# GIJaws/gym-simpletetris

Measured on AMD Instinct MI355X. Metric: env-steps/sec at 65 536 parallel 10×20 boards; 1→8 GPU scaling, higher is better.
Workload: dtype u32

## Files before the change

gym-simpletetris_amd/csrc/st_kernels.hip:

```cpp
#include "st_internal.h"


namespace st {
namespace {

constexpr int kShapes[7][4][2] = {
    {{0, 0}, {-1, 0}, {1, 0}, {0, -1}},   {{0, 0}, {-1, 0}, {0, -1}, {0, -2}},
    {{0, 0}, {1, 0}, {0, -1}, {0, -2}},   {{0, 0}, {-1, 0}, {0, -1}, {1, -1}},
    {{0, 0}, {-1, -1}, {0, -1}, {1, 0}},  {{0, 0}, {0, -1}, {0, -2}, {0, -3}},
    {{0, 0}, {0, -1}, {-1, 0}, {-1, -1}},
};

struct PieceTab {
    uint32_t m[28], g[28];
    bool ok;
};

constexpr PieceTab make_piece_tab() {
    PieceTab t{};
    t.ok = true;
    for (int p = 0; p < 7; ++p) {
        int cx[4] = {}, cy[4] = {};
        for (int c = 0; c < 4; ++c) {
            cx[c] = kShapes[p][c][0];
// ... 30 lines not shown
                const int i = cx[c], j = cy[c];
                cx[c] = j;
                cy[c] = -i;
            }
        }
    }
    return t;
}
constexpr PieceTab kTab = make_piece_tab();
static_assert(kTab.ok, "every tetromino column must be a contiguous run within [-3, 3]");
#define ST_TAB28(a) {a[0], a[1], a[2], a[3], a[4], a[5], a[6], a[7], a[8], a[9], a[10], a[11], \
                     a[12], a[13], a[14], a[15], a[16], a[17], a[18], a[19], a[20], a[21], a[22], \
                     a[23], a[24], a[25], a[26], a[27]}
__constant__ uint32_t c_tab_m[28] = ST_TAB28(kTab.m);
__constant__ uint32_t c_tab_g[28] = ST_TAB28(kTab.g);

constexpr PieceTab make_box_tab() {
    PieceTab t{};
    t.ok = true;
    for (int p = 0; p < 7; ++p) {
        int cx[4] = {}, cy[4] = {};
        for (int c = 0; c < 4; ++c) {
            cx[c] = kShapes[p][c][0];
            cy[c] = kShapes[p][c][1];
        }
        for (int r = 0; r < 4; ++r) {
            int dx0 = 99, dx1 = -99;
            for (int c = 0; c < 4; ++c) {
                dx0 = cx[c] < dx0 ? cx[c] : dx0;
                dx1 = cx[c] > dx1 ? cx[c] : dx1;
            }
            if (dx0 < -3 || dx0 > 0 || dx1 - dx0 > 3) t.ok = false;
            uint32_t m = 0, g = (uint32_t)(dx0 + 3);
            for (int k = 0; k < 4; ++k) g |= 64u << (3 + 7 * k);
            for (int k = 0; k < 4; ++k) {
                int ymin = 99, ymax = -99, cnt = 0;
                uint32_t bits = 0;
                for (int c = 0; c < 4; ++c)
                    if (cx[c] == dx0 + k) {
                        ++cnt;
                        ymin = cy[c] < ymin ? cy[c] : ymin;
                        ymax = cy[c] > ymax ? cy[c] : ymax;
                        bits |= 1u << (cy[c] + 3);
                    }
                if (!cnt) continue;
                if (cnt != ymax - ymin + 1 || ymin < -3 || ymax > 3) t.ok = false;
                m |= bits << (8 * k);
                g = (g & ~(127u << (3 + 7 * k))) | ((uint32_t)(ymax + 1) & 127u) << (3 + 7 * k);
            }
            t.m[p * 4 + r] = m;
            t.g[p * 4 + r] = g;
            for (int c = 0; c < 4; ++c) {
                const int i = cx[c], j = cy[c];
                cx[c] = j;
                cy[c] = -i;
            }
        }
    }
    return t;
}
constexpr PieceTab kBox = make_box_tab();
static_assert(kBox.ok, "every rotation must span at most four columns from dx0 in [-3, 0]");

__device__ __forceinline__ int pc_dx(uint32_t g, int j) { return (int)((g >> (6 * j)) & 7u) - 3; }
__device__ __forceinline__ int pc_bot(uint32_t g, int j) { return (int)((g >> (6 * j + 3)) & 7u) - 3; }
template <bool S32 = false>
__device__ __forceinline__ uint32_t pc_bits(uint32_t m, int j, int y) {
    if constexpr (S32) return (((m >> (8 * j)) & 0xFFu) << y) >> 3;
    return (uint32_t)((uint64_t)((m >> (8 * j)) & 0xFFu) << y >> 3);
}

typedef int i32x4 __attribute__((ext_vector_type(4)));
constexpr uint32_t kOff = 0xFFFFFFF0u;
__device__ __forceinline__ __amdgpu_buffer_rsrc_t buf_rsrc(const void *base, uint32_t bytes) {
    return __builtin_amdgcn_make_buffer_rsrc(const_cast<void *>(base), 0, base ? (int)bytes : 0,
                                             0x00020000);
}
constexpr int kNT = 2;
constexpr int kST = kNT;
constexpr int kRD = kNT;
constexpr int kDrawPrio = 2;
constexpr int kLogicPrio = 1;
template <int AUX = 0>
__device__ __forceinline__ void buf_store16(__amdgpu_buffer_rsrc_t r, uint32_t off, uint4 v) {
    const i32x4 d = {(int)v.x, (int)v.y, (int)v.z, (int)v.w};
    __builtin_amdgcn_raw_buffer_store_b128(d, r, off, 0, AUX);
}

__device__ __forceinline__ uint32_t &lcol(uint32_t *L, int x, int lane) {
    return L[(x + kPad) * kWave + lane];
}

__device__ __forceinline__ void read_cols(const uint32_t *L, int lane, uint32_t g, int x,
                                          uint32_t (&v)[4]) {
#pragma unroll
    for (int j = 0; j < 4; ++j) v[j] = L[(x + pc_dx(g, j) + kPad) * kWave + lane];
}
template <bool S32 = false>
__device__ __forceinline__ bool collides_v(uint32_t m, int y, const uint32_t (&v)[4]) {
    uint32_t hit = 0;
#pragma unroll
    for (int j = 0; j < 4; ++j) hit |= pc_bits<S32>(m, j, y) & v[j];
    return hit != 0;
}
__device__ __forceinline__ int drop_v(uint32_t g, int y, const uint32_t (&v)[4]) {
    int dist = 1 << 20;
#pragma unroll
    for (int j = 0; j < 4; ++j) {
        const int yb = y + pc_bot(g, j);
        const int s = yb + 1 > 0 ? yb + 1 : 0;
        const int k = __builtin_ctz(v[j] & (~0u << s)) - yb - 1;
        dist = k < dist ? k : dist;
    }
    return dist;
}

template <bool S32 = false>
__device__ __forceinline__ void paint(uint32_t *L, int lane, uint32_t m, uint32_t g, int x, int y,
                                      uint32_t hmask) {
#pragma unroll
    for (int j = 0; j < 4; ++j)
        atomicOr(&L[(x + pc_dx(g, j) + kPad) * kWave + lane], pc_bits<S32>(m, j, y) & hmask);
}

template <bool S32 = false>
__device__ __forceinline__ void erase(uint32_t *L, int lane, uint32_t m, uint32_t g, int x, int y,
                                      uint32_t hmask) {
#pragma unroll
    for (int j = 0; j < 4; ++j)
        atomicAnd(&L[(x + pc_dx(g, j) + kPad) * kWave + lane], ~(pc_bits<S32>(m, j, y) & hmask));
}

__device__ __forceinline__ int box_x0(uint32_t g, int x) { return x + (int)(g & 7u) - 3; }
__device__ __forceinline__ void read_box(const uint32_t *L, int lane, uint32_t g, int x, uint32_t (&v)[4]) {
    const uint32_t *c0 = &L[(box_x0(g, x) + kPad) * kWave + lane];
#pragma unroll
    for (int j = 0; j < 4; ++j) v[j] = c0[j * kWave];
}
__device__ __forceinline__ int drop_box(uint32_t g, int y, const uint32_t (&v)[4]) {
    int dist = 0;
#pragma unroll
    for (int j = 0; j < 4; ++j) {
        const int q = y + ((int32_t)(g << (32 - 10 - 7 * j)) >> 25);
        const int s = q > 0 ? q : 0;
        const int k = __builtin_ctz(v[j] & (~0u << s)) - q;
        dist = j == 0 || k < dist ? k : dist;
    }
    return dist;
}
template <bool S32 = false>
__device__ __forceinline__ void paint_box(uint32_t *L, int lane, uint32_t m, uint32_t g, int x, int y,
                                          uint32_t hmask) {
    uint32_t *c0 = &L[(box_x0(g, x) + kPad) * kWave + lane];
#pragma unroll
    for (int j = 0; j < 4; ++j) atomicOr(&c0[j * kWave], pc_bits<S32>(m, j, y) & hmask);
}
template <bool S32 = false>
__device__ __forceinline__ void erase_box(uint32_t *L, int lane, uint32_t m, uint32_t g, int x, int y,
                                          uint32_t hmask) {
    uint32_t *c0 = &L[(box_x0(g, x) + kPad) * kWave + lane];
#pragma unroll
    for (int j = 0; j < 4; ++j) atomicAnd(&c0[j * kWave], ~(pc_bits<S32>(m, j, y) & hmask));
}

__device__ __forceinline__ uint32_t compact(uint32_t v, uint32_t full) {
    while (full) {
        const int r = __builtin_ctz(full);
        full &= full - 1u;
        const uint32_t above = (1u << r) - 1u;
        v = (v & ~(above | (1u << r))) | ((v & above) << 1);
    }
    return v;
}

__device__ __forceinline__ void wave_sync() {
    __builtin_amdgcn_fence(__ATOMIC_RELEASE, "wavefront");
    __builtin_amdgcn_wave_barrier();
    __builtin_amdgcn_fence(__ATOMIC_ACQUIRE, "wavefront");
}

__device__ __forceinline__ uint32_t mt_temper(uint32_t y) {
    y ^= (y >> 11);
    y = __builtin_amdgcn_bitop3_b32(y, y << 7, 0x9d2c5680u, 0x78);
    y = __builtin_amdgcn_bitop3_b32(y, y << 15, 0xefc60000u, 0x78);
    y ^= (y >> 18);
    return y;
}
__device__ __forceinline__ uint32_t mt_temper_hi18(uint32_t y) {
    y ^= (y >> 11);
    y = __builtin_amdgcn_bitop3_b32(y, y << 7, 0x9d2c5680u, 0x78);
    return __builtin_amdgcn_bitop3_b32(y, y << 15, 0xefc60000u, 0x78);
}
__device__ __forceinline__ uint32_t mt_mix(uint32_t a, uint32_t b) {
    const uint32_t y = (a & 0x80000000u) | (b & 0x7fffffffu);
    return (y >> 1) ^ ((y & 1u) ? 0x9908b0dfu : 0u);
}

constexpr uint32_t kMtB = kMtN;
constexpr uint32_t kMtPad = 2 * kMtN;
constexpr int kMtWin = 16;
__device__ __forceinline__ void mt_unpack(uint32_t r, int &idx, int &pg, int &cur) {
    idx = (int)(r & 0x3FFu);
    pg = (int)((r >> 10) & 0x3FFu);
    cur = (int)((r >> 20) & 1u);
}
__device__ __forceinline__ uint32_t mt_pack(int idx, int pg, int cur) {
    return (uint32_t)idx | ((uint32_t)pg << 10) | ((uint32_t)cur << 20);
}
constexpr uint32_t kMtLow = (1u << 21) - 1u;
constexpr uint32_t kPvOk = 1u << 24;
constexpr uint32_t kPvCMax = 63u;
__device__ __forceinline__ uint32_t mt_keep(uint32_t hi, uint32_t low) { return (hi & ~kMtLow) | low; }
__device__ __forceinline__ int pv_id(uint32_t r) { return (int)((r >> 21) & 7u); }
// ... 445 lines not shown
    [[maybe_unused]] uint64_t draw_kind = 0;
    constexpr bool S32 = HT != 0 && HT <= 25;
    const uint32_t kFlags = SC0 ? (p.flags & (ST_REWARD_STEP | ST_STEP_RESET)) : p.flags;

#if defined(ST_ABLATION) && ST_ABLATION
    const uint32_t kAblate = p.ablate;
#else
    constexpr uint32_t kAblate = 0u;
#endif
    [[maybe_unused]] uint64_t rt0 = 0;
    if constexpr (STAMP) {
        rt0 = __builtin_amdgcn_s_memrealtime();
        tlast = __builtin_amdgcn_s_memtime();
    }
    ST_STAMP(0);
    if constexpr (ROLE == kRoleL && KSTEPS == 1) __builtin_amdgcn_s_setprio(kLogicPrio);
    uint32_t *const L = sm.L;
    uint32_t *const SS = sm.SS;
    const int W = WT ? WT : p.W;
    const int H = HT ? HT : p.H;
    const int lane = threadIdx.x & (kWave - 1);
    const int64_t e0 = (int64_t)blockIdx.x * kWave;
    const int64_t e = e0 + lane;
    const int64_t sd = p.stride;
    const bool real = e < p.n;
    const uint32_t hmask = (1u << H) - 1u;
    const uint32_t floorb = ~hmask;

    const uint32_t loff = (uint32_t)(lane >> 4) * (uint32_t)sd + 4u * (uint32_t)(lane & 15);
    constexpr int NBQ = ((WT ? WT : kMaxW) + 3) / 4;
    const uint32_t *bsrc = p.board + e0;
    const uint32_t *ssrc = reinterpret_cast<const uint32_t *>(p.stats) + ((kAblate & 1024u) ? 0 : e0);
    constexpr bool OVP = KSTEPS == 1;
    constexpr bool LCL = KSTEPS == 1 && !VEC;
    static_assert(ST_STAT_MT_INDEX == ST_STAT_COUNT0 + 7, "counts and MT word: 8 consecutive rows");
    auto mine_q = [&](int q) {
        if constexpr (LCL) return ROLE == kRoleD && (q == 1 || q == 2);
        return (ROLE == kRoleL) == (q < 2);
    };
    auto qbase = [&](int q) -> int {
        if constexpr (LCL) return ST_STAT_COUNT0 + 4 * (q - 1);
        return 4 * q;
    };
    auto clamp_off = [&](int q, int nrows) -> uint32_t {
        const int r = 4 * q + (lane >> 4) < nrows ? (lane >> 4) : nrows - 1 - 4 * q;
        return (uint32_t)r * (uint32_t)sd + 4u * (uint32_t)(lane & 15);
    };
    uint4 bv[NBQ];
    if constexpr (DO_L) {
#pragma unroll
        for (int q = 0; q < NBQ; ++q)
            if (WT || 4 * q < W)
                bv[q] = *reinterpret_cast<const uint4 *>(bsrc + (size_t)(4 * q) * sd +
                                                         (4 * q + 4 <= W ? loff : clamp_off(q, W)));
    }
    static_assert(kHotQ == 4, "four staged counter groups");
    uint4 sv0 = make_uint4(0u, 0u, 0u, 0u), sv1 = sv0, sv2 = sv0, sv3 = sv0;
    auto ldq = [&](int q) -> uint4 {
        return *reinterpret_cast<const uint4 *>(ssrc + (size_t)qbase(q) * sd +
                                                (qbase(q) + 4 <= kHotRows ? loff : clamp_off(q, kHotRows)));
    };
    if (mine_q(0)) sv0 = ldq(0);
    if (mine_q(1) && !(LCL && (kAblate & 262144u))) sv1 = ldq(1);
    if (mine_q(2)) sv2 = ldq(2);
    if (mine_q(3)) sv3 = ldq(3);
    const int K = KSTEPS ? KSTEPS : p.k;
    constexpr bool STEP2 = KSTEPS == 1;
    constexpr bool ACT = DO_L;
    uint32_t act_next = 0;
    if constexpr (ACT) act_next = p.actions[real ? e : p.n - 1];
    [[maybe_unused]] uint32_t gate_v = 0;
    if constexpr (VEC) gate_v = __builtin_amdgcn_raw_buffer_load_b32(buf_rsrc(p.gate, 4u), 0u, 0, 0);
    constexpr bool DL = KSTEPS == 1 && ROLE == kRoleL;
    [[maybe_unused]] uint32_t pw_d = 0, tm_d = 0;
    if constexpr (DL) {
        pw_d = p.piece[e];
        tm_d = reinterpret_cast<const uint32_t *>(p.stats)[(int64_t)ST_STAT_TIME * sd + e];
    }
    constexpr bool BUILD = DO_D;
    uint32_t tab_m = 0, tab_g = 0;
    if constexpr (BUILD) {
#pragma unroll
        for (int i = 0; i < 28; ++i) {
            asm("v_writelane_b32 %0, %1, %2" : "+v"(tab_m) : "s"(kTab.m[i]), "i"(i));
            asm("v_writelane_b32 %0, %1, %2" : "+v"(tab_g) : "s"(kTab.g[i]), "i"(i));
        }
    }
    const int lrow = lane >> 4, lcc = 4 * (lane & 15);
    if constexpr (DO_L) {
#pragma unroll
        for (int q = 0; q < NBQ; ++q) {
            if (WT || 4 * q < W) {
                uint4 v = bv[q];
                v.x |= floorb;
                v.y |= floorb;
                v.z |= floorb;
                v.w |= floorb;
                uint32_t *dst = &L[(4 * q + lrow + kPad) * kWave + lcc];
                if constexpr (ROLE == kRoleL) dst = 4 * q + lrow < W ? dst : &sm.dump[lcc];
                *reinterpret_cast<uint4 *>(dst) = v;
            }
        }
    }
    if constexpr (BUILD) {
#pragma unroll
        for (int x = 0; x < kPad; ++x) {
            L[x * kWave + lane] = ~0u;
            L[(W + kPad + x) * kWave + lane] = ~0u;
        }
        if (lane < 28) {
            sm.T2[2 * lane] = tab_m;
            sm.T2[2 * lane + 1] = tab_g;
        }
        if constexpr (F32) {
            if (lane < 16) {
                sm.F4[4 * lane] = (float)(lane & 1);
                sm.F4[4 * lane + 1] = (float)((lane >> 1) & 1);
                sm.F4[4 * lane + 2] = (float)((lane >> 2) & 1);
                sm.F4[4 * lane + 3] = (float)((lane >> 3) & 1);
            }
        }
    }
    auto stq = [&](int q, const uint4 &v) { *reinterpret_cast<uint4 *>(&SS[(qbase(q) + lrow) * kWave + lcc]) = v; };
    if (mine_q(0)) stq(0, sv0);
    if (mine_q(1)) stq(1, sv1);
    if (mine_q(2)) stq(2, sv2);
    if (mine_q(3)) stq(3, sv3);
    if constexpr (OVP && DO_L) {
#pragma unroll
        for (int q = 0; q < NBQ; ++q)
            if ((WT || 4 * q < W) && 4 * q + lrow < W)
                *reinterpret_cast<uint4 *>(&sm.OV[(4 * q + lrow + kPad) * kWave + lcc]) = make_uint4(0u, 0u, 0u, 0u);
    }
    if (ROLE == kRoleL && lane == 0) sm.f1 = 0u;
    if (ROLE == kRoleD && lane == 0) sm.f2 = 0u;
    wg_barrier();
    if constexpr (VEC) {
        if (p.gate && __builtin_amdgcn_readfirstlane(gate_v) == p.gate_epoch) return;
    }
    auto ss = [&](int r) -> uint32_t & { return SS[r * kWave + lane]; };
    auto tab = [&](int i) -> uint2 { return *reinterpret_cast<const uint2 *>(&sm.T2[2 * i]); };
    [[maybe_unused]] bool bad_act = false;
    for (int t = 0; t < K; ++t) {
    uint32_t act = 6u;
    if constexpr (ACT) {
        act = real ? act_next : 6u;
        bad_act |= act > 6u;
        if (KSTEPS != 1 && t + 1 < K) act_next = p.actions[(int64_t)(t + 1) * p.n + (real ? e : p.n - 1)];
    }
    uint32_t *const obs_t = p.obs ? p.obs + (int64_t)t * W * p.n : nullptr;
    const uint32_t pw = DL ? pw_d : ss(kPieceRow);
    int32_t time = (int32_t)(DL ? tm_d : ss(ST_STAT_TIME));
    const int id = (int)(pw & 7u);
    int rot = (int)((pw >> 3) & 3u);
    int ax = (int)((pw >> 5) & 63u);
    int ay = (int)((pw >> 11) & 63u);
    int lock = (int)(pw >> 17);
    uint32_t mt0 = ss(ST_STAT_MT_INDEX);
    if constexpr (STAMP && KSTEPS == 1) asm volatile("s_waitcnt vmcnt(0) lgkmcnt(0)" ::: "memory");
    ST_STAMP(1);

    uint2 desc = make_uint2(0u, 0u);
    bool locknow = false;
    int32_t rew = 0;
    [[maybe_unused]] uint2 pd_pv = make_uint2(0u, 0u);
    if constexpr (ACT) {
        const bool tries = act == 0u || act == 1u || act == 4u || act == 5u;
        const int cx = ax + (act == 0u ? -1 : (act == 1u ? 1 : 0));
        const int cr = (rot + (act == 4u ? 1 : 0) + (act == 5u ? 3 : 0)) & 3;
        desc = tab(id * 4 + rot);
        const uint2 cdesc = tab(id * 4 + cr);
        if constexpr (OVP && DO_L) pd_pv = tab(pv_id(mt0) * 4);
        uint32_t cur[4], cand[4];
        read_cols(L, lane, desc.y, ax, cur);
        read_cols(L, lane, cdesc.y, cx, cand);
        const bool ok = tries && !collides_v<S32>(cdesc.x, ay, cand);
        ax = ok ? cx : ax;
        rot = ok ? cr : rot;
        desc.x = ok ? cdesc.x : desc.x;
        desc.y = ok ? cdesc.y : desc.y;
#pragma unroll
        for (int j = 0; j < 4; ++j) cur[j] = ok ? cand[j] : cur[j];
        int d = drop_v(desc.y, ay, cur);
        if (act == 2u) {
            ay += d;
            d = 0;
        } else if (act == 3u && d > 0) {
            ay += 1;
            d -= 1;
        }
        if (d > 0) {
            ay += 1;
            d -= 1;
            if (kFlags & ST_STEP_RESET) lock = 0;
        }
        time += 1;
        rew = (kFlags & ST_REWARD_STEP) ? 1 : 0;
        if (d == 0) {
            const int l1 = lock + 1;
            lock = lock_next(l1, p.lock_mod);
            locknow = lock == 0 && !(kAblate & 1u);
        }
    }
    ST_STAMP(2);
    [[maybe_unused]] uint32_t lcv[5] = {};
    if constexpr (LCL && DO_L) {
        const auto rs = buf_rsrc(p.stats, (uint32_t)kHotRows * (uint32_t)sd * 4u);
        const uint32_t eo = (kAblate & 8192u) ? (uint32_t)lane * 4u : (uint32_t)e * 4u;
#pragma unroll
        for (int j = 0; j < 5; ++j)
            lcv[j] = __builtin_amdgcn_raw_buffer_load_b32(
                rs, locknow && !(kAblate & 2097152u) ? eo + (uint32_t)(ST_STAT_SCORE + j) * (uint32_t)sd * 4u : kOff,
                0, 0);
    }
    [[maybe_unused]] MtChunk chunk;
    [[maybe_unused]] MtRes mrs;
    [[maybe_unused]] int32_t cnt[7];
    [[maybe_unused]] DrawPar dpar;
    [[maybe_unused]] int32_t csid = 0;
    if constexpr (DO_D) {
        mrs = mt_res(p.mt + e0 * kMtPitch, lane);
        mt_chunk_issue(mrs, mt0, real && !(kAblate & (2u | 1048576u)), lane, chunk);
        const int s0 = pv_id(mt0);
#pragma unroll
        for (int i = 0; i < 7; ++i) cnt[i] = (int32_t)ss(ST_STAT_COUNT0 + i) + (i == s0);
        csid = cnt[0];
#pragma unroll
        for (int i = 1; i < 7; ++i) csid = s0 == i ? cnt[i] : csid;
        dpar = draw_par(cnt);
    }
    if constexpr (DO_L) {
        const uint64_t m = __ballot(locknow);
        if (lane == 0) {
            sm.lockm[t & 1][0] = (uint32_t)m;
            sm.lockm[t & 1][1] = (uint32_t)(m >> 32);
        }
    }
    wg_barrier();
    if constexpr (DO_D || KSTEPS != 1) ST_STAMP(10);
    if constexpr (DO_D) __builtin_amdgcn_s_setprio(kDrawPrio);
    if constexpr (DO_D) {
        const uint32_t w = lane < 32 ? sm.lockm[t & 1][0] : sm.lockm[t & 1][1];
        locknow = (w >> (lane & 31)) & 1u;
    }
    if constexpr (DO_L && KSTEPS != 1) {
        if (t > 0) mt0 = sm.mtw[(t - 1) & 1][lane];
    }

    uint32_t mtst = mt0;
    const bool want_pre = locknow && !(kAblate & 2u);
    constexpr int kWin = STEP2 ? 8 : 16;
    MtPre pre;
    if constexpr (DO_D) mt_pre_load<kWin>(mrs, mtst, want_pre && !(kAblate & 524288u), pre);

    [[maybe_unused]] const bool wide_obs1 = OVP && (p.n & 3) == 0 && e0 + kWave <= p.n &&
                                            (reinterpret_cast<uintptr_t>(p.obs) & 15u) == 0 &&
                                            (!VEC || (reinterpret_cast<uintptr_t>(p.final_obs) & 15u) == 0);

    bool died = false, spawn = false;
    int32_t score = 0, lines = 0, holes = 0, height = 0, deaths = 0;
    int32_t o_score = 0, o_lines = 0, o_holes = 0, o_height = 0, o_deaths = 0;
    [[maybe_unused]] bool hset = false;
    uint32_t bdirty = 0;
    if (DO_L && locknow) {
        if constexpr (!LCL) {
            score = o_score = (int32_t)ss(ST_STAT_SCORE);
            lines = o_lines = (int32_t)ss(ST_STAT_LINES);
            holes = o_holes = (int32_t)ss(ST_STAT_HOLES);
            height = o_height = (int32_t)ss(ST_STAT_PIECE_HEIGHT);
            deaths = o_deaths = (int32_t)ss(ST_STAT_DEATHS);
        }
        paint<S32>(L, lane, desc.x, desc.y, ax, ay, hmask);
        uint32_t andv = ~0u, orv = 0, sctz = 0, spop = 0;
        [[maybe_unused]] uint32_t cw[WT ? WT : 1];
        if constexpr (WT != 0) {
#pragma unroll
            for (int x = 0; x < WT; ++x) cw[x] = lcol(L, x, lane);
            __builtin_amdgcn_sched_barrier(0);
#pragma unroll
            for (int x = 0; x < WT; ++x) {
                const uint32_t v = cw[x];
                andv &= v;
                orv |= v;
                sctz += __builtin_ctz(v);
                spop += __builtin_popcount(v);
            }
        } else {
#pragma unroll 8
            for (int x = 0; x < W; ++x) {
                const uint32_t v = lcol(L, x, lane);
                andv &= v;
                orv |= v;
                sctz += __builtin_ctz(v);
                spop += __builtin_popcount(v);
            }
        }
        andv &= hmask;
        if constexpr (KSTEPS == 1) {
#pragma unroll
            for (int j = 0; j < 4; ++j) bdirty |= 1u << (ax + pc_dx(desc.y, j));
            if (andv) bdirty = ~0u;
        }
        int32_t ncl = 0;
        if (andv) {
            ncl = __builtin_popcount(andv);
            orv = 0;
            sctz = spop = 0;
            if constexpr (WT != 0) {
                uint32_t c[WT];
#pragma unroll
                for (int x = 0; x < WT; ++x) c[x] = cw[x] & hmask;
                uint32_t full = andv;
                while (full) {
                    const int r = __builtin_ctz(full);
                    full &= full - 1u;
                    const uint32_t above = (1u << r) - 1u;
                    const uint32_t keep = ~(above | (1u << r));
#pragma unroll
                    for (int x = 0; x < WT; ++x) c[x] = (c[x] & keep) | ((c[x] & above) << 1);
                }
#pragma unroll
                for (int x = 0; x < WT; ++x) {
                    const uint32_t v = c[x] | floorb;
                    lcol(L, x, lane) = v;
                    orv |= v;
                    sctz += __builtin_ctz(v);
                    spop += __builtin_popcount(v);
                }
            } else {
#pragma unroll 8
                for (int x = 0; x < W; ++x) {
                    const uint32_t v = compact(lcol(L, x, lane) & hmask, andv) | floorb;
                    lcol(L, x, lane) = v;
                    orv |= v;
                    sctz += __builtin_ctz(v);
                    spop += __builtin_popcount(v);
                }
            }
            lines += ncl;
        }
        orv &= hmask;
        const int32_t nh = W * H - (int32_t)sctz - ((int32_t)spop - W * (32 - H));
        if (kFlags & ST_ADVANCED_CLEARS) {
            constexpr uint64_t kClr = (40ull << 12) | (100ull << 24) | (300ull << 36) | (1200ull << 48);
            const int32_t sc = ncl <= 4 ? (int32_t)((kClr >> (12 * ncl)) & 0xFFFu) : 0;
            rew += (sc * 5) / 2;
            score += sc;
        } else if (kFlags & ST_HIGH_SCORING) {
            rew += 1000 * ncl;
            score += ncl;
        } else {
            rew += 100 * ncl;
            score += ncl;
        }
        if (orv & 1u) {
            holes = nh;
            deaths += 1;
            died = true;
            rew = -100;
        } else {
            const int32_t old_holes = LCL ? 0 : holes;
            holes = nh;
            const int32_t hgt = __builtin_popcount(orv);
            if (kFlags & ST_PENALISE_HEIGHT) {
                rew -= hgt;
            } else if (kFlags & ST_PENALISE_HEIGHT_INCREASE) {
                const int32_t oh = LCL ? (int32_t)lcv[3] : height;
                if (hgt > oh) rew -= 10 * (hgt - oh);
                height = hgt;
                hset = true;
            }
            if (kFlags & ST_PENALISE_HOLES) rew -= 5 * holes;
            else if (kFlags & ST_PENALISE_HOLES_INCREASE) rew -= 5 * (holes - (LCL ? (int32_t)lcv[2] : old_holes));
            spawn = true;
        }
    }
    ST_STAMP(3);

    const bool reset_now = died && p.autoreset == ST_AUTORESET_SAME_STEP;
    bool draw = spawn || reset_now;
    if (DO_L && p.autoreset != ST_AUTORESET_SAME_STEP) {
        const uint64_t m = __ballot(draw);
        if (lane == 0) {
            sm.drawm[0] = (uint32_t)m;
            sm.drawm[1] = (uint32_t)(m >> 32);
            lds_flag_set(&sm.f1, (uint32_t)t + 1u);
        }
    }
    uint2 odesc = desc;
    int oax = ax, oay = ay;
    if constexpr (DO_L) {
        const auto rr = buf_rsrc(p.reward ? p.reward + (int64_t)t * p.n : nullptr, (uint32_t)p.n * 4u);
        const auto rd = buf_rsrc(p.done ? p.done + (int64_t)t * p.n : nullptr, (uint32_t)p.n);
        __builtin_amdgcn_raw_buffer_store_b32(rew, rr, real ? (uint32_t)e * 4u : kOff, 0, kRD);
        __builtin_amdgcn_raw_buffer_store_b8((char)(died ? 1 : 0), rd, real ? (uint32_t)e : kOff, 0, kRD);
        if constexpr (KSTEPS == 1) ST_STAMP(10);
    }
    if constexpr (DO_L && KSTEPS == 1) {
        if (died && !reset_now) erase<S32>(L, lane, desc.x, desc.y, ax, ay, hmask);
        if (died) bdirty = ~0u;
        if constexpr (OVP) {
            uint2 pd = pd_pv;
            const bool need1 = draw && !pv_ok(mt0);
            if (__ballot(need1)) {
                lds_flag_wait(&sm.f2, (uint32_t)t + 1u);
                if (need1) pd = tab((int)sm.pick1[lane] * 4);
            }
            const uint32_t om = spawn ? pd.x : desc.x, og = spawn ? pd.y : desc.y;
            const int ox = spawn ? W / 2 : ax, oy = spawn ? 0 : ay;
#pragma unroll
            for (int j = 0; j < 4; ++j)
                if (!(kAblate & 4194304u)) sm.OV[(ox + pc_dx(og, j) + kPad) * kWave + lane] = pc_bits<S32>(om, j, oy) & hmask;
        }
        uint4 km, bd4;
        uint4 bw[NBQ], ow[NBQ];
        if (kAblate & 4194304u) {
            km = make_uint4(hmask, hmask, hmask, hmask);
            bd4 = make_uint4(bdirty, bdirty, bdirty, bdirty);
#pragma unroll
            for (int q = 0; q < NBQ; ++q) {
                bw[q] = make_uint4(bdirty, (uint32_t)ax, (uint32_t)ay, (uint32_t)lane);
                ow[q] = make_uint4(desc.x, desc.y, (uint32_t)rew, (uint32_t)q);
            }
        } else {
        sm.KM[lane] = reset_now ? 0u : hmask;
        sm.BD[lane] = bdirty;
        wave_sync();
        km = *reinterpret_cast<const uint4 *>(&sm.KM[lcc]);
        bd4 = *reinterpret_cast<const uint4 *>(&sm.BD[lcc]);
#pragma unroll
        for (int q = 0; q < NBQ; ++q) {
            if (WT || 4 * q < W) {
                bw[q] = *reinterpret_cast<const uint4 *>(&L[(4 * q + lrow + kPad) * kWave + lcc]);
                if constexpr (OVP) ow[q] = *reinterpret_cast<const uint4 *>(&sm.OV[(4 * q + lrow + kPad) * kWave + lcc]);
            }
        }
        }
        __builtin_amdgcn_sched_barrier(0);
        asm volatile("" : "+v"(km.x), "+v"(km.y), "+v"(km.z), "+v"(km.w), "+v"(bd4.x), "+v"(bd4.y), "+v"(bd4.z),
                     "+v"(bd4.w));
        if constexpr (STAMP) {
            asm volatile("s_waitcnt lgkmcnt(0)" ::: "memory");
            ST_STAMP(11);
        }
        const uint32_t bdl = (bd4.x | bd4.y | bd4.z | bd4.w) >> lrow;
        const auto rb = buf_rsrc(p.board, (uint32_t)W * (uint32_t)sd * 4u);
        const uint32_t boff = ((uint32_t)e0 * 4u + loff * 4u);
        [[maybe_unused]] const auto ro = buf_rsrc(wide_obs1 ? p.obs : nullptr, (uint32_t)W * (uint32_t)p.n * 4u);
        [[maybe_unused]] const auto rf = buf_rsrc(VEC && wide_obs1 ? p.final_obs : nullptr,
                                                  (uint32_t)W * (uint32_t)p.n * 4u);
#pragma unroll
        for (int q = 0; q < NBQ; ++q) {
            if (WT || 4 * q < W) {
                uint4 v = bw[q];
                if constexpr (OVP) {
                    const uint4 o = ow[q];
                    const uint4 ob = make_uint4((v.x | o.x) & hmask, (v.y | o.y) & hmask, (v.z | o.z) & hmask,
                                                (v.w | o.w) & hmask);
                    const uint32_t ooff =
                        ((uint32_t)e0 + (uint32_t)(4 * q + lrow) * (uint32_t)p.n + (uint32_t)lcc) * 4u;
                    if constexpr (VEC) {
                        const bool fin = !(km.x && km.y && km.z && km.w);
                        buf_store16<kNT>(rf, fin ? ooff : kOff, ob);
                        const uint4 keep = p.final_obs ? km : make_uint4(~0u, ~0u, ~0u, ~0u);
                        buf_store16<kNT>(ro, ooff, make_uint4(ob.x & keep.x, ob.y & keep.y, ob.z & keep.z, ob.w & keep.w));
                    } else {
                        buf_store16<kNT>(ro, ooff, ob);
                    }
                }
                v.x &= km.x;
                v.y &= km.y;
                v.z &= km.z;
                v.w &= km.w;
                const bool dirty = ((bdl >> (4 * q)) & 1u) && 4 * q + lrow < W && !(kAblate & 4096u);
                buf_store16<kST>(rb, dirty ? boff + (uint32_t)(4 * q) * (uint32_t)sd * 4u : kOff, v);
            }
        }
    }

    ST_STAMP(8);
    int sid = pv_id(mt0);
    if constexpr (DO_D) {
        const bool dr_spec = locknow;
        if constexpr (STAMP) {
            asm volatile("s_waitcnt vmcnt(0)" ::: "memory");
            ST_STAMP(9);
        }
        [[maybe_unused]] const uint32_t mt_before = mtst;
        uint32_t mt_new = mtst;
        if (!(kAblate & 2u)) {
            mt_win_consume<kWin>(pre);
            const bool need1 = dr_spec && !pv_ok(mt0);
            if (__ballot(need1)) {
                int32_t c0[7];
#pragma unroll
                for (int i = 0; i < 7; ++i) c0[i] = (int32_t)ss(ST_STAT_COUNT0 + i);
                const int pk = draw_shape<kWin, false>(need1, c0, mtst, p.mt + e0 * kMtPitch, sm.S, lane, pre, false);
                if (need1) {
                    sid = pk;
#pragma unroll
                    for (int i = 0; i < 7; ++i) cnt[i] = c0[i] + (i == pk);
#pragma unroll
                    for (int i = 0; i < 7; ++i) csid = pk == i ? cnt[i] : csid;
                }
                dpar = draw_par(cnt);
            }
            sm.pick1[lane] = (uint32_t)sid;
            if (lane == 0) lds_flag_set(&sm.f2, (uint32_t)t + 1u);
            const uint32_t m0 = mtst;
            const int npv = draw_core<kWin>(dr_spec, dpar, mtst, p.mt + e0 * kMtPitch, sm.S, lane, pre,
                                            want_pre && pv_ok(mt0));
            mt_new = pv_pack(mtst, npv, mt_consumed(m0, mtst));
        } else {
            sm.pick1[lane] = (uint32_t)sid;
            if (lane == 0) lds_flag_set(&sm.f2, (uint32_t)t + 1u);
        }
        const int chunk_pg = mt_chunk_store<KSTEPS == 1 ? kST : 0>(mrs, lane, chunk);
        const bool chunk_me = lane == chunk.l;
        ST_STAMP(4);
        if constexpr (STAMP) {
            const int i0 = (int)(mt_before & 0x3FFu), i1 = (int)(mt_new & 0x3FFu);
            draw_kind = (__ballot(dr_spec && i1 < i0) ? 1u : 0u) | (__ballot(dr_spec && i1 >= i0 && i1 - i0 > 8) ? 2u : 0u);
        }
        bool dr = draw;
        dr = locknow;
        if (p.autoreset != ST_AUTORESET_SAME_STEP) {
            lds_flag_wait(&sm.f1, (uint32_t)t + 1u);
            const uint32_t w = lane < 32 ? sm.drawm[0] : sm.drawm[1];
            dr = (w >> (lane & 31)) & 1u;
        }
        uint32_t mt_out = dr ? mt_new : mt0;
        if (chunk_me && (mt_out & (1u << 20)) == (mt0 & (1u << 20))) {
            int i2, pg2, c2;
            mt_unpack(mt_out, i2, pg2, c2);
            mt_out = mt_keep(mt_out, mt_pack(i2, chunk_pg, c2));
        }
        if constexpr (STEP2) {
            const auto rs = buf_rsrc(p.stats, (uint32_t)kHotRows * (uint32_t)sd * 4u);
            const uint32_t eo = (uint32_t)e * 4u;
            const bool cst = !(kAblate & (2048u | 32768u));
            const bool mst = cst && !(kAblate & 131072u) && (dr || chunk_me);
            const bool kst = cst && !(kAblate & 65536u) && dr;
            __builtin_amdgcn_raw_buffer_store_b32(mt_out, rs, mst ? eo + (uint32_t)ST_STAT_MT_INDEX * (uint32_t)sd * 4u : kOff,
                                                  0, kST);
            __builtin_amdgcn_raw_buffer_store_b32(
                (uint32_t)csid, rs, kst ? eo + (uint32_t)(ST_STAT_COUNT0 + sid) * (uint32_t)sd * 4u : kOff, 0, kST);
            if constexpr (VEC) {
                const auto ri = buf_rsrc(p.info, (uint32_t)ST_NSTAT * (uint32_t)p.n * 4u);
#pragma unroll
                for (int i = 0; i < 7; ++i)
                    __builtin_amdgcn_raw_buffer_store_b32(
                        (uint32_t)(dr ? cnt[i] : (int32_t)ss(ST_STAT_COUNT0 + i)), ri,
                        real ? ((uint32_t)(ST_STAT_COUNT0 + i) * (uint32_t)p.n + (uint32_t)e) * 4u : kOff, 0, kNT);
            }
        } else {
            if (dr || chunk_me) ss(ST_STAT_MT_INDEX) = mt_out;
            if (dr) atomicAdd(&ss(ST_STAT_COUNT0 + sid), 1u);
            sm.mtw[t & 1][lane] = mt_out;
        }
        ST_STAMP(11);
    }

    if constexpr (DO_L) {
        const bool need1 = draw && !pv_ok(mt0);
        if (__ballot(need1)) {
            lds_flag_wait(&sm.f2, (uint32_t)t + 1u);
            if (need1) sid = (int)sm.pick1[lane];
        }
        ST_STAMP(4);
        uint32_t pw_out = pack_piece(id, rot, ax, ay, lock);
        if (draw) pw_out = pack_piece(sid, 0, W / 2, 0, lock);
        if (spawn) {
            odesc = tab(sid * 4);
            oax = W / 2;
            oay = 0;
        }

        if constexpr (LCL) {
            if (locknow) {
                o_score = (int32_t)lcv[0];
                o_lines = (int32_t)lcv[1];
                o_holes = (int32_t)lcv[2];
                o_height = (int32_t)lcv[3];
                o_deaths = (int32_t)lcv[4];
                score += o_score;
                lines += o_lines;
                deaths += o_deaths;
                if (!hset) height = o_height;
            }
        }
        [[maybe_unused]] int32_t ep_t = 0, ep_s = 0, ep_l = 0, ep_h = 0;
        if constexpr (VEC) {
            if (reset_now) {
                ep_t = time;
                ep_s = score;
                ep_l = lines;
                ep_h = holes;
            }
        }
        if (reset_now) {
            int32_t *st = p.stats + e;
            st[ST_STAT_EP_TIME * sd] = time;
            st[ST_STAT_EP_SCORE * sd] = score;
            st[ST_STAT_EP_LINES * sd] = lines;
            st[ST_STAT_EP_HOLES * sd] = holes;
            time = score = lines = holes = height = 0;
        }
        if constexpr (STEP2) {
            const auto rs = buf_rsrc(p.stats, (uint32_t)kHotRows * (uint32_t)sd * 4u);
            const uint32_t eo = (uint32_t)e * 4u;
            auto put = [&](int r, int32_t v, bool on) {
                __builtin_amdgcn_raw_buffer_store_b32((uint32_t)v, rs, on ? eo + (uint32_t)r * (uint32_t)sd * 4u : kOff,
                                                      0, kST);
            };
            put(ST_STAT_TIME, time, true);
            put(kPieceRow, (int32_t)pw_out, true);
            const bool cst = !(kAblate & (2048u | 16384u));
            put(ST_STAT_SCORE, score, cst && locknow && score != o_score);
            put(ST_STAT_LINES, lines, cst && locknow && lines != o_lines);
            put(ST_STAT_HOLES, holes, cst && locknow && holes != o_holes);
            put(ST_STAT_PIECE_HEIGHT, height, cst && locknow && height != o_height);
            put(ST_STAT_DEATHS, deaths, cst && locknow && deaths != o_deaths);
            if constexpr (VEC) {
                const auto ri = buf_rsrc(p.info, (uint32_t)ST_NSTAT * (uint32_t)p.n * 4u);
                const uint32_t io = (uint32_t)e * 4u;
                auto inf = [&](int r, int32_t v) {
                    __builtin_amdgcn_raw_buffer_store_b32((uint32_t)v, ri, real ? io + (uint32_t)r * (uint32_t)p.n * 4u : kOff,
                                                          0, kNT);
                };
                inf(ST_STAT_TIME, time);
                inf(kPieceRow, (int32_t)pw_out);
                inf(ST_STAT_SCORE, locknow ? score : (int32_t)ss(ST_STAT_SCORE));
                inf(ST_STAT_LINES, locknow ? lines : (int32_t)ss(ST_STAT_LINES));
                inf(ST_STAT_HOLES, locknow ? holes : (int32_t)ss(ST_STAT_HOLES));
                inf(ST_STAT_PIECE_HEIGHT, locknow ? height : (int32_t)ss(ST_STAT_PIECE_HEIGHT));
                inf(ST_STAT_DEATHS, locknow ? deaths : (int32_t)ss(ST_STAT_DEATHS));
                inf(ST_STAT_EP_TIME, ep_t);
                inf(ST_STAT_EP_SCORE, ep_s);
                inf(ST_STAT_EP_LINES, ep_l);
                inf(ST_STAT_EP_HOLES, ep_h);
            }
        } else {
            ss(ST_STAT_TIME) = (uint32_t)time;
            ss(kPieceRow) = pw_out;
            if (locknow) {
                auto put = [&](int r, int32_t v, int32_t) { ss(r) = (uint32_t)v; };
                put(ST_STAT_SCORE, score, o_score);
                put(ST_STAT_LINES, lines, o_lines);
                put(ST_STAT_HOLES, holes, o_holes);
                put(ST_STAT_PIECE_HEIGHT, height, o_height);
                put(ST_STAT_DEATHS, deaths, o_deaths);
            }
        }

        if constexpr (KSTEPS != 1) {
            if (KSTEPS != 1 || spawn) paint<S32>(L, lane, odesc.x, odesc.y, oax, oay, hmask);
        }
        wave_sync();
        const bool wide_obs = (p.n & 3) == 0 && e0 + kWave <= p.n &&
                              (reinterpret_cast<uintptr_t>(p.obs) & 15u) == 0 &&
                              (!VEC || (reinterpret_cast<uintptr_t>(p.final_obs) & 15u) == 0);
        if (obs_t && !(kAblate & 8u)) {
            if (OVP && wide_obs) {
            } else if (wide_obs) {
                const uint32_t noff = (uint32_t)lrow * (uint32_t)p.n + (uint32_t)lcc;
#pragma unroll
                for (int q = 0; q < NBQ; ++q) {
                    if ((WT || 4 * q < W) && 4 * q + lrow < W) {
                        uint4 v = *reinterpret_cast<const uint4 *>(&L[(4 * q + lrow + kPad) * kWave + lcc]);
                        v.x &= hmask;
                        v.y &= hmask;
                        v.z &= hmask;
                        v.w &= hmask;
                        buf_store16<kNT>(buf_rsrc(obs_t, (uint32_t)W * (uint32_t)p.n * 4u),
                                         ((uint32_t)e0 + (uint32_t)(4 * q) * (uint32_t)p.n + noff) * 4u, v);
                    }
                }
            } else if (real) {
                const auto ro = buf_rsrc(obs_t, (uint32_t)W * (uint32_t)p.n * 4u);
                const bool fin = VEC && p.final_obs && reset_now;
                const auto rf = buf_rsrc(VEC ? p.final_obs : nullptr, (uint32_t)W * (uint32_t)p.n * 4u);
#pragma unroll 1
                for (int x = 0; x < W; ++x) {
                    const uint32_t v = (lcol(L, x, lane) | (OVP ? lcol(sm.OV, x, lane) : 0u)) & hmask;
                    const uint32_t off = ((uint32_t)x * (uint32_t)p.n + (uint32_t)e) * 4u;
                    __builtin_amdgcn_raw_buffer_store_b32(fin ? 0u : v, ro, off, 0, kNT);
                    if constexpr (VEC) __builtin_amdgcn_raw_buffer_store_b32(v, rf, fin ? off : kOff, 0, kNT);
                }
            }
        }
        if constexpr (KSTEPS == 1) {
            if (p.wire) {
                const auto rw = buf_rsrc(p.wire, (uint32_t)((W * H + 33 + 31) / 32) * (uint32_t)p.n * 4u);
                uint32_t off = (uint32_t)e * 4u;
                const uint32_t rowb = (uint32_t)p.n * 4u;
                uint64_t acc = 0;
                int nb = 0;
                auto put = [&](uint32_t bits, int k) {
                    acc |= (uint64_t)bits << nb;
                    nb += k;
                    if (nb >= 32) {
                        __builtin_amdgcn_raw_buffer_store_b32((uint32_t)acc, rw, real ? off : kOff, 0, kNT);
                        off += rowb;
                        acc >>= 32;
                        nb -= 32;
                    }
                };
#pragma unroll
                for (int x = 0; x < (WT ? WT : kMaxW); ++x)
                    if (WT || x < W) put((lcol(L, x, lane) | lcol(sm.OV, x, lane)) & hmask, H);
                put((uint32_t)rew, 32);
                put(died ? 1u : 0u, 1);
                if (nb > 0) __builtin_amdgcn_raw_buffer_store_b32((uint32_t)acc, rw, real ? off : kOff, 0, kNT);
            }
        }
        if (F32) {
            const int64_t nreal64 = p.n - e0 < kWave ? p.n - e0 : kWave;
            const int nreal = (int)nreal64;
            float *out = p.obs_f32 + ((int64_t)t * p.n + e0) * (W * H);
            if constexpr (WT != 0 && HT % 4 == 0) {
                constexpr int CPC = HT / 4, CPE = WT * CPC;
                uint32_t *O = sm.O;
                const uint32_t omask = VEC && p.final_obs && reset_now ? 0u : hmask;
#pragma unroll
                for (int x = 0; x < WT; ++x)
                    O[lane * (WT + 1) + x] = (lcol(L, x, lane) | (OVP ? lcol(sm.OV, x, lane) : 0u)) & omask;
                wave_sync();
                float4 *out4 = reinterpret_cast<float4 *>(out);
                const float4 *F4 = reinterpret_cast<const float4 *>(sm.F4);
                const int total = nreal * CPE;
                for (int c = lane; c < total; c += kWave) {
                    const int ee = c / CPE;
                    const int cr = c - ee * CPE;
                    const int x = cr / CPC;
                    const int q = cr - x * CPC;
                    const float4 f = F4[(O[ee * (WT + 1) + x] >> (4 * q)) & 15u];
                    if constexpr (KSTEPS != 1) {
                        typedef float f32x4 __attribute__((ext_vector_type(4)));
                        const f32x4 fv = {f.x, f.y, f.z, f.w};
                        __builtin_nontemporal_store(fv, reinterpret_cast<f32x4 *>(&out4[c]));
                    } else {
                        out4[c] = f;
                    }
                }
            } else {
                const int per_env = W * H;
                const int total = nreal * per_env;
                auto word = [&](int ee, int x) {
                    return (L[(x + kPad) * kWave + ee] | (OVP ? sm.OV[(x + kPad) * kWave + ee] : 0u)) &
                           (VEC && p.final_obs ? sm.KM[ee] : hmask);
                };
                for (int f = lane; f < total; f += kWave) {
                    const int ee = f / per_env;
                    const int rem = f - ee * per_env;
                    const int x = rem / H;
                    const int y = rem - x * H;
                    out[f] = (float)((word(ee, x) >> y) & 1u);
                }
            }
        }
        ST_STAMP(5);

        if constexpr (KSTEPS != 1) {
            wave_sync();
            erase<S32>(L, lane, odesc.x, odesc.y, oax, oay, hmask);
            if (reset_now)
                for (int x = 0; x < W; ++x) lcol(L, x, lane) = floorb;
        }
    }
    }
    wave_sync();
    if constexpr (ACT) {
        __builtin_amdgcn_raw_buffer_store_b32(1u, buf_rsrc(p.act_flag, 4u), bad_act ? 0u : kOff, 0, 0);
    }
    if constexpr (KSTEPS != 1 && DO_L) {
        const auto rb = buf_rsrc(p.board, (uint32_t)((W + 3) & ~3) * (uint32_t)sd * 4u);
        const uint32_t boff = (uint32_t)e0 * 4u + loff * 4u;
#pragma unroll
        for (int q = 0; q < NBQ; ++q) {
            if (WT || 4 * q < W) {
                uint4 v = *reinterpret_cast<const uint4 *>(&L[(4 * q + lrow + kPad) * kWave + lcc]);
                v.x &= hmask;
                v.y &= hmask;
                v.z &= hmask;
                v.w &= hmask;
                buf_store16<kST>(rb, boff + (uint32_t)(4 * q) * (uint32_t)sd * 4u, v);
            }
        }
    }
    constexpr uint32_t kRowsD = ((1u << 7) - 1u) << ST_STAT_COUNT0 | 1u << ST_STAT_MT_INDEX;
    constexpr uint32_t kOwn = ROLE == kRoleD ? kRowsD : ((1u << kHotRows) - 1u) & ~kRowsD;
    const auto rs = buf_rsrc(p.stats, (uint32_t)kHotRows * (uint32_t)sd * 4u);
    const uint32_t soff = (uint32_t)e0 * 4u + loff * 4u;
#pragma unroll
    for (int q = 0; q < kHotQ; ++q) {
        if constexpr (STEP2) break;
        if (((kOwn >> (4 * q)) & 0xFu) == 0u) continue;
        const bool st = (kOwn >> (4 * q + lrow)) & 1u;
        buf_store16<kST>(rs, st ? soff + (uint32_t)(4 * q) * (uint32_t)sd * 4u : kOff,
                         *reinterpret_cast<const uint4 *>(&SS[(4 * q + lrow) * kWave + lcc]));
    }
    if constexpr (STAMP && KSTEPS != 1) {
        ST_STAMP(6);
        uint64_t *slot = p.stamps + (int64_t)blockIdx.x * kStampWords + (ROLE == kRoleD ? 16 : 0);
        if (lane == 0) {
#pragma unroll
            for (int i = 0; i < 12; ++i) slot[i] = tacc[i];
            slot[12] = __builtin_amdgcn_s_memrealtime() - rt0;
            slot[13] = (uint64_t)K;
        }
    }
    if constexpr (STAMP && KSTEPS == 1) {
        ST_STAMP(6);
        asm volatile("s_waitcnt vmcnt(0)" ::: "memory");
        ST_STAMP(7);
        uint64_t *slot = p.stamps + (int64_t)blockIdx.x * kStampWords + (ROLE == kRoleD ? 16 : 0);
        if (lane == 0) {
            if constexpr (ROLE == kRoleD) {
#pragma unroll
                for (int i = 0; i < 12; ++i) slot[i] = tstamp[i];
                slot[12] = rt0;
                slot[13] = __builtin_amdgcn_s_memrealtime();
                slot[14] = draw_kind;
            } else {
#pragma unroll
                for (int i = 0; i < 10; ++i) slot[i] = tstamp[i];
                slot[10] = rt0;
                slot[11] = __builtin_amdgcn_s_memrealtime();
                slot[12] = __builtin_amdgcn_s_getreg(0xF804);
                slot[13] = __builtin_amdgcn_s_getreg(0xF814);
                slot[14] = tstamp[10];
                slot[15] = tstamp[11];
            }
        }
    }
}

template <int WT, int HT, bool F32, bool STAMP = false, bool SC0 = false, bool VEC = false>
__global__ __launch_bounds__(2 * kWave) void k_step(uint32_t *board, int32_t *stats, const uint8_t *actions,
                                                    uint32_t *mt, int64_t stride, int64_t n, KParams p0) {
    KParams p = p0;
    p.board = board;
    p.stats = stats;
    p.actions = actions;
    p.mt = mt;
    p.stride = stride;
    p.n = n;
    __shared__ StepLds<WT, F32, 1> sm;
// ... 1608 lines not shown
```

Measured before the change: 14.61 billion.

## Switch piece ops to contiguous box-column tables and scalar buffer offsets

Replaces the per-cell column lookups (read_cols, drop_v, paint, erase) with box-based variants that read four consecutive LDS columns from a single base address. The build table moves from kTab to kBox, and the dirty-column mask is computed with a shift instead of a loop. Buffer loads and stores now pass row strides through the scalar offset operand rather than adding them per lane, which cuts VALU address arithmetic. The risk is that the box encoding must match every shape exactly, and paint_box/erase_box and kBox are assumed to be defined in the unshown code.

Measured after the change: 14.90 billion, median of 6. +2.0%, better.

```diff
diff --git a/gym-simpletetris_amd/csrc/st_kernels.hip b/gym-simpletetris_amd/csrc/st_kernels.hip
--- a/gym-simpletetris_amd/csrc/st_kernels.hip
+++ b/gym-simpletetris_amd/csrc/st_kernels.hip
@@ -136,20 +136,15 @@
 constexpr int kDrawPrio = 2;
 constexpr int kLogicPrio = 1;
 template <int AUX = 0>
-__device__ __forceinline__ void buf_store16(__amdgpu_buffer_rsrc_t r, uint32_t off, uint4 v) {
+__device__ __forceinline__ void buf_store16(__amdgpu_buffer_rsrc_t r, uint32_t off, uint4 v, uint32_t soff = 0u) {
     const i32x4 d = {(int)v.x, (int)v.y, (int)v.z, (int)v.w};
-    __builtin_amdgcn_raw_buffer_store_b128(d, r, off, 0, AUX);
+    __builtin_amdgcn_raw_buffer_store_b128(d, r, off, soff, AUX);
 }
 
 __device__ __forceinline__ uint32_t &lcol(uint32_t *L, int x, int lane) {
     return L[(x + kPad) * kWave + lane];
 }
 
-__device__ __forceinline__ void read_cols(const uint32_t *L, int lane, uint32_t g, int x,
-                                          uint32_t (&v)[4]) {
-#pragma unroll
-    for (int j = 0; j < 4; ++j) v[j] = L[(x + pc_dx(g, j) + kPad) * kWave + lane];
-}
 template <bool S32 = false>
 __device__ __forceinline__ bool collides_v(uint32_t m, int y, const uint32_t (&v)[4]) {
     uint32_t hit = 0;
@@ -175,14 +170,6 @@
 #pragma unroll
     for (int j = 0; j < 4; ++j)
         atomicOr(&L[(x + pc_dx(g, j) + kPad) * kWave + lane], pc_bits<S32>(m, j, y) & hmask);
-}
-
-template <bool S32 = false>
-__device__ __forceinline__ void erase(uint32_t *L, int lane, uint32_t m, uint32_t g, int x, int y,
-                                      uint32_t hmask) {
-#pragma unroll
-    for (int j = 0; j < 4; ++j)
-        atomicAnd(&L[(x + pc_dx(g, j) + kPad) * kWave + lane], ~(pc_bits<S32>(m, j, y) & hmask));
 }
 
 __device__ __forceinline__ int box_x0(uint32_t g, int x) { return x + (int)(g & 7u) - 3; }
@@ -794,8 +781,8 @@
     if constexpr (BUILD) {
 #pragma unroll
         for (int i = 0; i < 28; ++i) {
-            asm("v_writelane_b32 %0, %1, %2" : "+v"(tab_m) : "s"(kTab.m[i]), "i"(i));
-            asm("v_writelane_b32 %0, %1, %2" : "+v"(tab_g) : "s"(kTab.g[i]), "i"(i));
+            asm("v_writelane_b32 %0, %1, %2" : "+v"(tab_m) : "s"(kBox.m[i]), "i"(i));
+            asm("v_writelane_b32 %0, %1, %2" : "+v"(tab_g) : "s"(kBox.g[i]), "i"(i));
         }
     }
     const int lrow = lane >> 4, lcc = 4 * (lane & 15);
@@ -884,8 +871,8 @@
         const uint2 cdesc = tab(id * 4 + cr);
         if constexpr (OVP && DO_L) pd_pv = tab(pv_id(mt0) * 4);
         uint32_t cur[4], cand[4];
-        read_cols(L, lane, desc.y, ax, cur);
-        read_cols(L, lane, cdesc.y, cx, cand);
+        read_box(L, lane, desc.y, ax, cur);
+        read_box(L, lane, cdesc.y, cx, cand);
         const bool ok = tries && !collides_v<S32>(cdesc.x, ay, cand);
         ax = ok ? cx : ax;
         rot = ok ? cr : rot;
@@ -893,7 +880,7 @@
         desc.y = ok ? cdesc.y : desc.y;
 #pragma unroll
         for (int j = 0; j < 4; ++j) cur[j] = ok ? cand[j] : cur[j];
-        int d = drop_v(desc.y, ay, cur);
+        int d = drop_box(desc.y, ay, cur);
         if (act == 2u) {
             ay += d;
             d = 0;
@@ -919,11 +906,10 @@
     if constexpr (LCL && DO_L) {
         const auto rs = buf_rsrc(p.stats, (uint32_t)kHotRows * (uint32_t)sd * 4u);
         const uint32_t eo = (kAblate & 8192u) ? (uint32_t)lane * 4u : (uint32_t)e * 4u;
+        const uint32_t lo = locknow && !(kAblate & 2097152u) ? eo : kOff;
 #pragma unroll
         for (int j = 0; j < 5; ++j)
-            lcv[j] = __builtin_amdgcn_raw_buffer_load_b32(
-                rs, locknow && !(kAblate & 2097152u) ? eo + (uint32_t)(ST_STAT_SCORE + j) * (uint32_t)sd * 4u : kOff,
-                0, 0);
+            lcv[j] = __builtin_amdgcn_raw_buffer_load_b32(rs, lo, (uint32_t)(ST_STAT_SCORE + j) * (uint32_t)sd * 4u, 0);
     }
     [[maybe_unused]] MtChunk chunk;
     [[maybe_unused]] MtRes mrs;
@@ -982,7 +968,7 @@
             height = o_height = (int32_t)ss(ST_STAT_PIECE_HEIGHT);
             deaths = o_deaths = (int32_t)ss(ST_STAT_DEATHS);
         }
-        paint<S32>(L, lane, desc.x, desc.y, ax, ay, hmask);
+        paint_box<S32>(L, lane, desc.x, desc.y, ax, ay, hmask);
         uint32_t andv = ~0u, orv = 0, sctz = 0, spop = 0;
         [[maybe_unused]] uint32_t cw[WT ? WT : 1];
         if constexpr (WT != 0) {
@@ -1009,8 +995,7 @@
         }
         andv &= hmask;
         if constexpr (KSTEPS == 1) {
-#pragma unroll
-            for (int j = 0; j < 4; ++j) bdirty |= 1u << (ax + pc_dx(desc.y, j));
+            bdirty = (0xFu >> (__builtin_clz(desc.x) >> 3)) << box_x0(desc.y, ax);
             if (andv) bdirty = ~0u;
         }
         int32_t ncl = 0;
@@ -1109,7 +1094,7 @@
         if constexpr (KSTEPS == 1) ST_STAMP(10);
     }
     if constexpr (DO_L && KSTEPS == 1) {
-        if (died && !reset_now) erase<S32>(L, lane, desc.x, desc.y, ax, ay, hmask);
+        if (died && !reset_now) erase_box<S32>(L, lane, desc.x, desc.y, ax, ay, hmask);
         if (died) bdirty = ~0u;
         if constexpr (OVP) {
             uint2 pd = pd_pv;
@@ -1120,9 +1105,10 @@
             }
             const uint32_t om = spawn ? pd.x : desc.x, og = spawn ? pd.y : desc.y;
             const int ox = spawn ? W / 2 : ax, oy = spawn ? 0 : ay;
+            uint32_t *const ov0 = &sm.OV[(box_x0(og, ox) + kPad) * kWave + lane];
 #pragma unroll
             for (int j = 0; j < 4; ++j)
-                if (!(kAblate & 4194304u)) sm.OV[(ox + pc_dx(og, j) + kPad) * kWave + lane] = pc_bits<S32>(om, j, oy) & hmask;
+                if (!(kAblate & 4194304u)) ov0[j * kWave] = pc_bits<S32>(om, j, oy) & hmask;
         }
         uint4 km, bd4;
         uint4 bw[NBQ], ow[NBQ];
@@ -1185,7 +1171,7 @@
                 v.z &= km.z;
                 v.w &= km.w;
                 const bool dirty = ((bdl >> (4 * q)) & 1u) && 4 * q + lrow < W && !(kAblate & 4096u);
-                buf_store16<kST>(rb, dirty ? boff + (uint32_t)(4 * q) * (uint32_t)sd * 4u : kOff, v);
+                buf_store16<kST>(rb, dirty ? boff : kOff, v, (uint32_t)(4 * q) * (uint32_t)sd * 4u);
             }
         }
     }
@@ -1322,8 +1308,8 @@
             const auto rs = buf_rsrc(p.stats, (uint32_t)kHotRows * (uint32_t)sd * 4u);
             const uint32_t eo = (uint32_t)e * 4u;
             auto put = [&](int r, int32_t v, bool on) {
-                __builtin_amdgcn_raw_buffer_store_b32((uint32_t)v, rs, on ? eo + (uint32_t)r * (uint32_t)sd * 4u : kOff,
-                                                      0, kST);
+                __builtin_amdgcn_raw_buffer_store_b32((uint32_t)v, rs, on ? eo : kOff, (uint32_t)r * (uint32_t)sd * 4u,
+                                                      kST);
             };
             put(ST_STAT_TIME, time, true);
             put(kPieceRow, (int32_t)pw_out, true);
@@ -1366,7 +1352,7 @@
         }
 
         if constexpr (KSTEPS != 1) {
-            if (KSTEPS != 1 || spawn) paint<S32>(L, lane, odesc.x, odesc.y, oax, oay, hmask);
+            if (KSTEPS != 1 || spawn) paint_box<S32>(L, lane, odesc.x, odesc.y, oax, oay, hmask);
         }
         wave_sync();
         const bool wide_obs = (p.n & 3) == 0 && e0 + kWave <= p.n &&
@@ -1475,7 +1461,7 @@
 
         if constexpr (KSTEPS != 1) {
             wave_sync();
-            erase<S32>(L, lane, odesc.x, odesc.y, oax, oay, hmask);
+            erase_box<S32>(L, lane, odesc.x, odesc.y, oax, oay, hmask);
             if (reset_now)
                 for (int x = 0; x < W; ++x) lcol(L, x, lane) = floorb;
         }
```
